# JCBrouwer/maua-style

Measured on AMD Instinct MI355X. Metric: optimizer iterations/sec at 1024x1024 VGG-19, higher is better.
Workload: dtype f32 (fp16x3 split-precision MFMA, fp32 accumulate)

## Files before the change

maua-style_amd/csrc/conv_x3p.hip:

```cpp
#include <stdlib.h>

#include <type_traits>

#include "conv_host.hpp"
#include "fp16x3.hpp"

namespace maua {

constexpr int XP_COT = 64;
constexpr int XP_ROWS = 16, XP_PR = 18, XP_PC = 34;
constexpr int XP_NPOS = XP_PR * XP_PC;
constexpr int XP_NPOS_PAD = 624;
constexpr int XP_PLANE = XP_NPOS_PAD * 16;
constexpr int XP_PATCH_BYTES = 8 * XP_PLANE;
constexpr int XP_TAP_BYTES = 2 * 4 * XP_COT * 16;
constexpr int XP_W_BYTES = 9 * XP_TAP_BYTES;
constexpr int XP_NI = 5;
constexpr int XP_THREADS = 512;
constexpr int XP_BIAS_MAX = 512;
constexpr int XP_LDS_BYTES = XP_PATCH_BYTES + XP_W_BYTES + 64 + XP_BIAS_MAX * 4 + XP_THREADS * 12;
constexpr unsigned XP_OOB = 0x80000000u;
#ifndef XP_W1_PIECES
#define XP_W1_PIECES 4
#endif
#ifndef XP_EARLY_LOADS
#define XP_EARLY_LOADS 0
#endif
#ifndef XP_MIDFOLD
#define XP_MIDFOLD 1
#endif
#ifndef XP_STAGGER
#define XP_STAGGER 0
#endif

__host__ __device__ constexpr int xp_first_pieces(bool pool) { return pool ? XP_W1_PIECES / 2 : XP_W1_PIECES; }
__host__ __device__ constexpr int xp_step_of(bool pool, int k) {
    const int p1 = xp_first_pieces(pool);
    return pool ? (k < p1 ? 16 - 2 * (p1 - 1 - k) : 20 + 2 * (k - p1)) : (k < p1 ? 17 - p1 + k : 20 + (k - p1));
}

struct X3pArgs {
    int items;
    int tiles;
    int ncot;
    int ksplit;
    int cps;
    int nmain;
    int n2;
    int groups;
    int tiles_y;
    int d_split, d_tx, d_ty, d_cot, d_n;
    int order;
    float w_inv_scale;
};

#ifdef XP_STAMP
#define XP_MARK(k)                                                                                                       \
    do {                                                                                                                 \
        if (lane == 0 && p.mask && chunk_no < 60) {                                                                      \
            const_cast<float*>(p.mask)[(((int64_t)blockIdx.x * 8 + wave) * 64 + chunk_no) * 8 + (k)] =                   \
                __builtin_bit_cast(float, (unsigned)__builtin_amdgcn_s_memtime());                                       \
        }                                                                                                                \
    } while (0)
#else
#define XP_MARK(k) do {} while (0)
#endif

#define XP_FENCE() __builtin_amdgcn_sched_barrier(0)

#define XP_PIPE_PLAIN(VA)                                             \
    do {                                                              \
        _Pragma("unroll") for (int m_ = 0; m_ < 12; ++m_) {           \
            __builtin_amdgcn_sched_group_barrier(0x008, 1, 0);        \
            __builtin_amdgcn_sched_group_barrier(0x100, 1, 0);        \
            __builtin_amdgcn_sched_group_barrier(0x020, 1, 0);        \
            __builtin_amdgcn_sched_group_barrier(0x200, 1, 0);        \
            __builtin_amdgcn_sched_group_barrier(0x002, VA, 0);       \
        }                                                             \
    } while (0)
#define XP_PIPE(VA)                                                   \
    do {                                                              \
        _Pragma("unroll") for (int m_ = 0; m_ < 12; ++m_) {           \
            __builtin_amdgcn_sched_group_barrier(0x008, 1, 0);        \
            __builtin_amdgcn_sched_group_barrier(0x100, 1, 0);        \
            __builtin_amdgcn_sched_group_barrier(0x020, 1, 0);        \
            __builtin_amdgcn_sched_group_barrier(0x040, 1, 0);        \
// ... 309 lines not shown
#pragma unroll
        for (int part = 0; part < 2; ++part) af[buf][part] = *reinterpret_cast<const f16x8*>(Wl + a_base + (tap * 2 + part) * 4096 + i * 256);
    };
    auto step_ = [&](auto stores, int tap, int i, int next_tap, auto fresh, float inv, auto va, auto&& extra) {
        constexpr bool FRESH = decltype(fresh)::value;
        constexpr int VA = decltype(va)::value;
        const int cur = i & 1;
        const bool refresh = i == 3 && next_tap >= 0;
        XP_FENCE();
        if (i < 3) load_ai(cur ^ 1, tap, i + 1);
        else if (next_tap >= 0 && tap != 4) load_ai(cur ^ 1, next_tap, 0);
        const f32x4 zero = {0.f, 0.f, 0.f, 0.f};
        if constexpr (FRESH) {
#pragma unroll
            for (int g = 0; g < 4; ++g) asm volatile("" : "+v"(acc[i][g]));
#pragma unroll
            for (int g = 0; g < 4; ++g)
#pragma unroll
                for (int r = 0; r < 4; ++r) master[i][g][r] = fmaf(acc[i][g][r], inv, master[i][g][r]);
#pragma unroll
            for (int g = 0; g < 4; ++g) asm volatile("" : "+v"(master[i][g]));
        }
#pragma unroll
        for (int g = 0; g < 4; ++g) acc[i][g] = __builtin_amdgcn_mfma_f32_16x16x32_f16(af[cur][1], bf[g][0], FRESH ? zero : acc[i][g], 0, 0, 0);
#pragma unroll
        for (int g = 0; g < 4; ++g) {
            acc[i][g] = __builtin_amdgcn_mfma_f32_16x16x32_f16(af[cur][0], bf[g][0], acc[i][g], 0, 0, 0);
            if (refresh) load_bg(g, 0, next_tap);
        }
        extra();
#pragma unroll
        for (int g = 0; g < 4; ++g) {
            acc[i][g] = __builtin_amdgcn_mfma_f32_16x16x32_f16(af[cur][0], bf[g][1], acc[i][g], 0, 0, 0);
            if (refresh) load_bg(g, 1, next_tap);
        }
        if constexpr (decltype(stores)::value) XP_PIPE(VA);
        else XP_PIPE_PLAIN(VA);
        XP_FENCE();
    };
    auto nothing = []() {};
    constexpr std::true_type FOLD{};
    constexpr std::false_type KEEP{};
    constexpr std::integral_constant<int, 0> V0{};
    constexpr std::integral_constant<int, 2> V2{};
    constexpr std::integral_constant<int, 4> V4{};

    Item cur = decode(item_begin);
    Item fin = cur;
    bool fin_valid = false;
    __amdgpu_buffer_rsrc_t rs_out, rs_aux;
    unsigned so_base = 0;
    unsigned vo[2];
    bool row_ok[4] = {true, true, true, true};
    const int PW = p.OW >> 1;
    const int pplane = (p.OH >> 1) * PW;
    auto epi_begin = [&]() {
        const int t_ = my_tid();
        const int lane = t_ & 63, px = t_ & 15, oct = (t_ >> 4) & 3, wave = wv;
        if constexpr (POOL) {
            const int64_t img = (int64_t)fin.n * p.Cout * pplane;
            rs_out = __builtin_amdgcn_make_buffer_rsrc(p.y + img, 0, (unsigned)p.Cout * (unsigned)pplane * 4u, 0x00020000);
            rs_aux = __builtin_amdgcn_make_buffer_rsrc(p.pool_codes + img, 0, (unsigned)p.Cout * (unsigned)pplane, 0x00020000);
            so_base = (unsigned)((fin.y0 >> 1) * PW + (fin.x0 >> 1));
#pragma unroll
            for (int h = 0; h < 2; ++h) {
                const int oy = fin.y0 + 2 * wave, oxx = fin.x0 + 16 * h + px;
                const bool store = fin_valid && (lane & 1) == 0 && oy + 1 < p.OH && oxx + 1 < p.OW;
                vo[h] = store ? (unsigned)(wave * PW + ((16 * h + px) >> 1)) : XP_OOB;
            }
        } else {
            const int64_t img = (int64_t)fin.n * p.Cout * out_plane;
            float* base = slab ? p.ws + ((int64_t)fin.n * ksplit + fin.split) * p.Cout * out_plane : p.y + img;
            rs_out = __builtin_amdgcn_make_buffer_rsrc(base, 0, (unsigned)p.Cout * (unsigned)out_plane * 4u, 0x00020000);
            rs_aux = rs_out;
            if constexpr (OM) rs_aux = __builtin_amdgcn_make_buffer_rsrc(const_cast<float*>(p.omask + img), 0, (unsigned)p.Cout * (unsigned)out_plane * 4u, 0x00020000);
            so_base = (unsigned)((fin.cot * XP_COT) * out_plane + fin.y0 * p.OW + fin.x0) * 4u;
#pragma unroll
            for (int h = 0; h < 2; ++h)
                vo[h] = fin_valid && fin.x0 + 16 * h + px < p.OW ? (unsigned)((4 * oct) * out_plane + (2 * wave) * p.OW + 16 * h + px) * 4u : XP_OOB;
#pragma unroll
            for (int g = 0; g < 4; ++g) row_ok[g] = fin.y0 + 2 * wv + (g >> 1) < p.OH;
        }
    };
    float mk[2][4];
    auto epi_load = [&](int k) {
        if constexpr (OM) {
            const int i = k >> 2, g = k & 3;
            const unsigned v = row_ok[g] ? vo[g & 1] : XP_OOB;
#pragma unroll
            for (int r = 0; r < 4; ++r)
                mk[k % 2][r] = __builtin_bit_cast(float, __builtin_amdgcn_raw_buffer_load_b32(
                    rs_aux, v, so_base + (unsigned)((16 * i + r) * out_plane + (g >> 1) * p.OW) * 4u, 0));
        }
    };
    auto reset_group = [&](int i, int cot) {
        const int oct = (my_tid() >> 4) & 3;
        const f32x4 b = *reinterpret_cast<const f32x4*>(Bl + cot * XP_COT + 16 * i + 4 * oct);
#pragma unroll
        for (int g = 0; g < 4; ++g) master[i][g] = b;
    };
    auto epi_piece = [&](int k, int next_cot) {
        const int oct = (my_tid() >> 4) & 3;
        if constexpr (POOL) {
            if (k >= 8) return;
            const int i = k >> 1, h = k & 1;
            unsigned pk = 0;
            const unsigned so = (unsigned)((fin.cot * XP_COT + 16 * i) * pplane) + so_base;
#pragma unroll
            for (int r = 0; r < 4; ++r) {
                float a = master[i][h][r], c = master[i][2 + h][r];
                a = a > 0.f ? a : 0.f;
                c = c > 0.f ? c : 0.f;
                const float b = __builtin_bit_cast(float, __builtin_amdgcn_update_dpp(0, __builtin_bit_cast(int, a), 0x101, 0xf, 0xf, false));
                const float d = __builtin_bit_cast(float, __builtin_amdgcn_update_dpp(0, __builtin_bit_cast(int, c), 0x101, 0xf, 0xf, false));
                float m = a;
                unsigned arg = 0;
                if (b > m) { m = b; arg = 1; }
                if (c > m) { m = c; arg = 2; }
                if (d > m) { m = d; arg = 3; }
                pk |= (arg | (m > 0.f ? 0u : 4u)) << (8 * r);
                const unsigned v = vo[h] == XP_OOB ? XP_OOB : ((unsigned)(4 * oct * pplane) + vo[h]) * 4u;
                __builtin_amdgcn_raw_buffer_store_b32(__builtin_bit_cast(unsigned, m), rs_out, v, (so + (unsigned)(r * pplane)) * 4u, 0);
            }
            const unsigned vc = vo[h] == XP_OOB ? XP_OOB : ((unsigned)((oct >> 1) * pplane) + vo[h]) * 8u + 4u * (oct & 1);
            __builtin_amdgcn_raw_buffer_store_b32(pk, rs_aux, vc, ((unsigned)(((fin.cot * XP_COT + 16 * i) >> 3) * pplane) + so_base) * 8u, 0);
            if (h == 1) reset_group(i, next_cot);
        } else {
            const int i = k >> 2, g = k & 3;
            const unsigned v = row_ok[g] ? vo[g & 1] : XP_OOB;
#pragma unroll
            for (int r = 0; r < 4; ++r) {
                float val = master[i][g][r];
                if (p.relu && !slab) val = val > 0.f ? val : 0.f;
                if constexpr (OM) val = mk[k % 2][r] > 0.f ? val : 0.f;
                __builtin_amdgcn_raw_buffer_store_b32(__builtin_bit_cast(unsigned, val), rs_out, v,
                                                      so_base + (unsigned)((16 * i + r) * out_plane + (g >> 1) * p.OW) * 4u, 0);
            }
            if (g == 3) reset_group(i, next_cot);
        }
    };

    auto gram_phase = [&](const Item& it, float inv_pending) {
#pragma unroll
        for (int i = 0; i < 4; ++i)
#pragma unroll
            for (int g = 0; g < 4; ++g)
#pragma unroll
                for (int r = 0; r < 4; ++r) {
                    master[i][g][r] = fmaf(acc[i][g][r], inv_pending, master[i][g][r]);
                    acc[i][g][r] = 0.f;
                }
        const float d_inv_scale = p.dinv[it.n];
        const unsigned char* dbank = reinterpret_cast<const unsigned char*>(p.dbank);
        unsigned vf[4];
#pragma unroll
        for (int g = 0; g < 4; ++g) {
            const int oy = it.y0 + 2 * wave + (g >> 1), oxx = it.x0 + (g & 1) * 16 + px;
            vf[g] = (oy < p.OH && oxx < p.OW) ? (unsigned)((oct * 8) * out_plane + oy * p.OW + oxx) * 4u : XP_OOB;
        }
        const unsigned frange = (unsigned)out_plane * 128u;
        float f[4][8];
        auto request = [&](int c2) {
            asm volatile("" : "+s"(c2));
            const __amdgpu_buffer_rsrc_t rs = __builtin_amdgcn_make_buffer_rsrc(
                const_cast<float*>(p.omask + ((int64_t)it.n * p.Cout + (int64_t)c2 * 32) * out_plane), 0, frange, 0x00020000);
#pragma unroll
            for (int c = 0; c < 8; ++c)
#pragma unroll
                for (int g = 0; g < 4; ++g) f[g][c] = __builtin_bit_cast(float, __builtin_amdgcn_raw_buffer_load_b32(rs, vf[g], c * out_plane * 4, 0));
        };
        request(0);
        for (int c2 = 0; c2 < q.n2; ++c2) {
            float m = 0.f;
#pragma unroll
            for (int g = 0; g < 4; ++g)
#pragma unroll
                for (int c = 0; c < 8; ++c) m = fmaxf(m, fabsf(f[g][c]));
            m = wave_max_nonneg(m);
            int e = (int)((__builtin_bit_cast(unsigned, m) >> 23) & 0xffu) - 127;
            e = m > 0.f ? max(e, -100) : 11;
            const float s = __builtin_bit_cast(float, (unsigned)(127 + 11 - e) << 23);
            const float inv = __builtin_bit_cast(float, (unsigned)(127 + e - 11) << 23) * d_inv_scale;
// ... 20 lines not shown
                for (int part = 0; part < 2; ++part) a[i][part] = *reinterpret_cast<const u32x4*>(gsrc + part * 2048 + i * 256);
            if (c2 + 1 < q.n2) request(c2 + 1);
#pragma unroll
            for (int i = 0; i < 4; ++i) {
                const f16x8 ah = __builtin_bit_cast(f16x8, a[i][0]), al = __builtin_bit_cast(f16x8, a[i][1]);
#pragma unroll
                for (int g = 0; g < 4; ++g) {
                    acc[i][g] = __builtin_amdgcn_mfma_f32_16x16x32_f16(al, b[g][0], acc[i][g], 0, 0, 0);
                    acc[i][g] = __builtin_amdgcn_mfma_f32_16x16x32_f16(ah, b[g][1], acc[i][g], 0, 0, 0);
                    acc[i][g] = __builtin_amdgcn_mfma_f32_16x16x32_f16(ah, b[g][0], acc[i][g], 0, 0, 0);
                }
            }
#pragma unroll
            for (int i = 0; i < 4; ++i)
#pragma unroll
                for (int g = 0; g < 4; ++g)
#pragma unroll
                    for (int r = 0; r < 4; ++r) {
                        master[i][g][r] = fmaf(acc[i][g][r], inv, master[i][g][r]);
                        acc[i][g][r] = 0.f;
                    }
        }
    };

    for (int c = tid; c < p.Cout; c += XP_THREADS) Bl[c] = (p.bias != nullptr && !slab) ? p.bias[c] : 0.f;
    set_tile(cur.x0, cur.y0);
    int ch = cur.cb;
    dma_filters(ch, cur.cot, 0, 9);
    if constexpr (!UNPOOL) voff[1] = Tl[2 * XP_THREADS + tid];
    load_patch_part(patch_rsrc(cur.n, ch), 0, 8);
    publish_max();
    asm volatile("s_waitcnt lgkmcnt(0)" ::: "memory");
    __builtin_amdgcn_s_barrier();
    float inv_prev = 0.f, inv_cur = 0.f, inv_next = 0.f;
    inv_cur = chunk_scale() * w_inv_scale;
    inv_next = inv_cur;
#pragma unroll
    for (int k = 0; k < NI; ++k) split_item(k);
    store_patch();
#pragma unroll
    for (int i = 0; i < 4; ++i) {
        reset_group(i, cur.cot);
#pragma unroll
        for (int g = 0; g < 4; ++g) acc[i][g] = f32x4{0.f, 0.f, 0.f, 0.f};
    }
    asm volatile("s_waitcnt vmcnt(0) lgkmcnt(0)" ::: "memory");
    __builtin_amdgcn_s_barrier();

#ifdef XP_STAMP
    int chunk_no = 0;
#endif
    auto chunk_body = [&](auto epi_tag, const Item& it, int chn, bool later, bool more, const Item& nx, int nch, const PatchSrc& rs) {
        constexpr bool EPI = decltype(epi_tag)::value;
        auto step = [&](int tap, int i, int next_tap, auto fresh, float inv, auto va, auto&& extra) {
            step_(std::integral_constant<bool, EPI>{}, tap, i, next_tap, fresh, inv, va, extra);
        };
        {
            const int t_ = my_tid();
            if constexpr (!UNPOOL) voff[1] = Tl[2 * XP_THREADS + t_];
            b_base = ((t_ >> 4) & 3) * XP_PLANE + ((2 * wv) * XP_PC + (t_ & 15)) * 16;
            a_base = ((t_ >> 4) & 3) * 1024 + (t_ & 15) * 16;
        }
        const int ncot_ = it.cot;
        if constexpr (EPI) epi_begin();
        constexpr int NP = POOL ? 8 : 16;
        constexpr int P1 = xp_first_pieces(POOL);
        auto step_of = [](int k) { return xp_step_of(POOL, k); };
        auto E = [&](int s) {
            if constexpr (EPI) {
#pragma unroll
                for (int k = 0; k < NP; ++k) {
                    if constexpr (OM) {
                        if (k < 1 ? s == step_of(0) - 1 : s == step_of(k - 1)) epi_load(k);
                    }
                }
#pragma unroll
                for (int k = 0; k < NP; ++k)
                    if (s == step_of(k) && fin_valid) epi_piece(k, ncot_);
            }
        };
        constexpr int SPP = POOL ? 5 : 4;
        constexpr int ST1 = !EPI ? 0 : SPP * P1;
        constexpr int late2 = POOL ? (NP - P1 > 3 ? NP - P1 - 3 : 0) : (NP - P1 > 5 ? NP - P1 - 5 : 0);
        constexpr int ST2 = !EPI ? 0 : SPP * late2;
        static_assert(ST1 <= 60 && ST2 <= 60 && xp_step_of(POOL, NP - 1) <= 31 && xp_step_of(POOL, 0) >= 5, "conv_x3p: epilogue schedule");
        constexpr std::integral_constant<int, EPI ? 4 : 2> VF{};
        constexpr std::integral_constant<int, EPI ? 2 : 0> VK{};
        XP_MARK(0);
#pragma unroll
        for (int g = 0; g < 4; ++g) {
            load_bg(g, 0, 0);
            load_bg(g, 1, 0);
        }
        load_ai(0, 0, 0);
        if constexpr (EPI || XP_EARLY_LOADS) {
            step(0, 0, 1, FOLD, inv_prev, VF, [&]() { load_patch_part(rs, 0, 1); });
            step(0, 1, 1, FOLD, inv_prev, VF, [&]() { load_patch_part(rs, 1, 2); if (later) dma_filters(chn, it.cot, 40, 1, 0); });
            step(0, 2, 1, FOLD, inv_prev, VF, [&]() { load_patch_part(rs, 2, 3); });
            step(0, 3, 1, FOLD, inv_prev, VF, [&]() { load_patch_part(rs, 3, 4); if (later) dma_filters(chn, it.cot, 40, 1, 1); });
            step(1, 0, 2, KEEP, 0.f, VK, [&]() { load_patch_part(rs, 4, 5); E(4); });
            step(1, 1, 2, KEEP, 0.f, VK, [&]() { load_patch_part(rs, 5, 6); if (later) dma_filters(chn, it.cot, 40, 1, 2); E(5); });
            step(1, 2, 2, KEEP, 0.f, VK, [&]() { load_patch_part(rs, 6, 7); E(6); });
            step(1, 3, 2, KEEP, 0.f, VK, [&]() { load_patch_part(rs, 7, 8); if (later) dma_filters(chn, it.cot, 40, 1, 3); E(7); });
#pragma unroll
            for (int tap = 2; tap < 4; ++tap)
#pragma unroll
                for (int i = 0; i < 4; ++i) step(tap, i, tap + 1, KEEP, 0.f, VK, [&]() { E(4 * tap + i); });
        } else {
            step(0, 0, 1, FOLD, inv_prev, VF, [&]() { load_patch_part(rs, 0, 1); });
            step(0, 1, 1, FOLD, inv_prev, VF, nothing);
            step(0, 2, 1, FOLD, inv_prev, VF, [&]() { load_patch_part(rs, 1, 2); });
            step(0, 3, 1, FOLD, inv_prev, VF, [&]() { if (later) dma_filters(chn, it.cot, 40, 1, 0); });
#pragma unroll
            for (int tap = 1; tap < 4; ++tap) {
                step(tap, 0, tap + 1, KEEP, 0.f, VK, [&]() { load_patch_part(rs, 2 * tap, 2 * tap + 1); });
                step(tap, 1, tap + 1, KEEP, 0.f, VK, nothing);
                step(tap, 2, tap + 1, KEEP, 0.f, VK, [&]() { load_patch_part(rs, 2 * tap + 1, 2 * tap + 2); });
                step(tap, 3, tap + 1, KEEP, 0.f, VK, [&]() { if (later) dma_filters(chn, it.cot, 40, 1, tap); });
            }
        }
        XP_MARK(1);
        step(4, 0, 5, KEEP, 0.f, VK, [&]() { E(16); });
        if (EPI && fin_valid) asm volatile("s_waitcnt vmcnt(%0)" ::"n"(ST1) : "memory");
        else asm volatile("s_waitcnt vmcnt(0)" ::: "memory");
        step(4, 1, 5, KEEP, 0.f, V4, [&]() { publish_max(); });
        step(4, 2, 5, KEEP, 0.f, V4, nothing);
        step(4, 3, 5, KEEP, 0.f, V0, nothing);
        XP_MARK(2);
        if (EPI && fin_valid) asm volatile("s_waitcnt vmcnt(%0) lgkmcnt(0)" ::"n"(ST1) : "memory");
        else asm volatile("s_waitcnt vmcnt(0) lgkmcnt(0)" ::: "memory");
        __builtin_amdgcn_s_barrier();
        XP_MARK(3);
        load_ai(0, 5, 0);
        inv_next = chunk_scale() * w_inv_scale;
// ... 35 lines not shown
        }
        XP_MARK(4);
        inv_prev = inv_cur;
        inv_cur = inv_next;
        asm volatile("s_waitcnt lgkmcnt(0)" ::: "memory");
        __builtin_amdgcn_s_barrier();
        XP_MARK(5);
        store_patch();
        if (EPI && fin_valid) asm volatile("s_waitcnt vmcnt(%0) lgkmcnt(0)" ::"n"(ST2) : "memory");
        else asm volatile("s_waitcnt vmcnt(0) lgkmcnt(0)" ::: "memory");
        __builtin_amdgcn_s_barrier();
        XP_MARK(6);
#ifdef XP_STAMP
        XP_MARK(7);
        ++chunk_no;
#endif
    };

    int item = item_begin;
    bool later = false;
    Item nx = cur;
    int nch = 0;
    bool more = true;
    PatchSrc rs;
    auto plan_next = [&](int chn) {
        const bool last_of_item = chn + 1 >= cur.ce;
        more = !(last_of_item && item + stride >= item_end);
        nx = cur;
        nch = chn + 1;
        if (last_of_item && more) {
            nx = advance(cur);
            nch = nx.cb;
            set_tile(nx.x0, nx.y0);
        }
        rs = patch_rsrc(more ? nx.n : cur.n, more ? nch : chn);
    };
    while (true) {
        plan_next(cur.cb);
        chunk_body(std::true_type{}, cur, cur.cb, later, more, nx, nch, rs);
        later = true;
        for (int chn = cur.cb + 1; chn < cur.ce; ++chn) {
            plan_next(chn);
            chunk_body(std::false_type{}, cur, chn, later, more, nx, nch, rs);
        }
        if constexpr (GRAM) {
            if (cur.split == ksplit - 1) {
                gram_phase(cur, inv_prev);
                inv_prev = 0.f;
            }
        }
        fin = cur;
        fin_valid = true;
        item += stride;
        if (!more) break;
        cur = nx;
    }
#pragma unroll
    for (int i = 0; i < 4; ++i)
#pragma unroll
        for (int g = 0; g < 4; ++g)
#pragma unroll
            for (int r = 0; r < 4; ++r) master[i][g][r] = fmaf(acc[i][g][r], inv_prev, master[i][g][r]);
    epi_begin();
    if constexpr (POOL) {
#pragma unroll
        for (int k = 0; k < 8; ++k) epi_piece(k, fin.cot);
    } else {
#pragma unroll
        for (int i = 0; i < 4; ++i) {
#pragma unroll
            for (int g = 0; g < 4; ++g) {
                epi_load(4 * i + g);
                epi_piece(4 * i + g, fin.cot);
            }
        }
    }
}


static int x3p_choose_split(const ConvArgs& a) {
    const int64_t items = conv_tiles(a, XP_ROWS) * ((a.Cout + XP_COT - 1) / XP_COT) * split_batch_hint();
    const int nchunks = a.Cin / 32;
    const int forced = (int)tuning("x3p_ks", 0);
    auto whole = [&](int ks) { const int cps = (nchunks + ks - 1) / ks; return (nchunks + cps - 1) / cps; };
    if (forced > 0) return whole(forced <= nchunks / 2 ? forced : (nchunks >= 4 ? nchunks / 2 : 1));
    if (items >= 512 || nchunks < 4) return 1;
    const double out_mb = (double)split_batch_hint() * a.Cout * a.OH * a.OW * 4.0 / 1e6;
    int best = 1;
    double best_cost = 1e30;
    for (int ks = 1; ks <= 16 && ks <= nchunks / 2; ++ks) {
        const int64_t its = items * ks;
        const double per_wg = (double)((its + 255) / 256);
        double cost = (per_wg * (double)((nchunks + ks - 1) / ks) + 0.7) * 9.0;
        if (ks > 1) cost += (ks + 1) * out_mb / 5.0 + 5.0;
        if (cost < best_cost * 0.97) {
            best_cost = cost;
            best = ks;
        }
    }
    return whole(best);
}

bool conv_x3p_supports(const ConvArgs& a) {
    return a.Cin % 32 == 0 && a.Cout % XP_COT == 0 && a.Cout <= XP_BIAS_MAX && (int64_t)a.H * a.W <= (1ll << 24) && a.pad >= 0 && a.pad <= 2 &&
           (int64_t)a.Cout * a.OH * a.OW * 4 < (1ll << 31) && (int64_t)a.OH * a.OW <= (1ll << 24);
}

static int g_xp_max_groups = 0;
static int x3p_max_groups() {
    const int v = g_xp_max_groups > 0 ? g_xp_max_groups : (int)tuning("x3p_groups", 256);
    return v >= 8 ? v / 8 * 8 : 256;
}

#ifdef XP_STAMP
static float* g_xp_stamp = nullptr;
extern "C" void maua_xp_set_stamp_buffer(float* buf) { g_xp_stamp = buf; }
#endif

template <bool OM, bool POOL, bool UNPOOL, bool GRAM>
static int xp_launch_one(const ConvArgs& p, const X3pArgs& q, hipStream_t stream) {
    const void* fn = reinterpret_cast<const void*>(&conv_x3p_kernel<OM, POOL, UNPOOL, GRAM>);
    static unsigned long long served = 0;
    const hipError_t rc = opt_in_dynamic_lds(fn, XP_LDS_BYTES, &served);
    if (rc != hipSuccess) {
        set_error("conv_x3p: hipFuncSetAttribute: %s", hipGetErrorString(rc));
        return (int)rc;
    }
    hipLaunchKernelGGL((conv_x3p_kernel<OM, POOL, UNPOOL, GRAM>), dim3((unsigned)q.groups), dim3(XP_THREADS), XP_LDS_BYTES, stream, p, q);
    return check_launch("conv_x3p_kernel");
// ... 146 lines not shown
```

maua-style_amd/csrc/conv_x3q.hip:

```cpp
#include <stdlib.h>

#include <type_traits>

#include "conv_host.hpp"
#include "fp16x3.hpp"

namespace maua {

constexpr int XQ_COT = 64;
constexpr int XQ_ROWS = 16, XQ_PR = 18, XQ_PC = 34;
constexpr int XQ_NPOS = XQ_PR * XQ_PC;
constexpr int XQ_NPOS_PAD = 624;
constexpr int XQ_PLANE = XQ_NPOS_PAD * 16;
constexpr int XQ_PATCH_BYTES = 8 * XQ_PLANE;
constexpr int XQ_TAP_BYTES = 2 * 4 * XQ_COT * 16;
constexpr int XQ_W_BYTES = 9 * XQ_TAP_BYTES;
constexpr int XQ_ITEMS = 4 * XQ_NPOS;
constexpr int XQ_NI = 5;
constexpr int XQ_THREADS = 512;
constexpr int XQ_LDS_BYTES = XQ_PATCH_BYTES + XQ_W_BYTES + 64;

__global__ void pack_x3q_kernel(const float* __restrict__ w, unsigned short* __restrict__ bank, int cout, int cin, int backward,
                                float w_scale) {
    const int CO = backward ? cin : cout;
    const int CI = backward ? cout : cin;
    const int nchunk = (CI + 31) / 32, ntile = (CO + XQ_COT - 1) / XQ_COT;
    const int64_t total = (int64_t)nchunk * ntile * 9 * 4 * XQ_COT * 8;
    for (int64_t e = (int64_t)blockIdx.x * blockDim.x + threadIdx.x; e < total; e += (int64_t)gridDim.x * blockDim.x) {
        int64_t r = e;
        const int ch = (int)(r % 8);
        r /= 8;
        const int co = (int)(r % XQ_COT);
        r /= XQ_COT;
        const int oct = (int)(r % 4);
        r /= 4;
        const int tap = (int)(r % 9);
        r /= 9;
        const int tile = (int)(r % ntile);
        const int chunk = (int)(r / ntile);
        const int o = tile * XQ_COT + co, i = chunk * 32 + oct * 8 + ch;
        float v = 0.f;
        if (o < CO && i < CI) {
            if (!backward) v = w[((int64_t)o * cin + i) * 9 + tap];
            else v = w[((int64_t)i * cin + o) * 9 + (8 - tap)];
        }
        v *= w_scale;
        const _Float16 h = (_Float16)v;
        const _Float16 l = (_Float16)(v - (float)h);
        const int64_t base = ((int64_t)chunk * ntile + tile) * (XQ_W_BYTES / 2);
        bank[base + ((((int64_t)tap * 2 + 0) * 4 + oct) * XQ_COT + co) * 8 + ch] = __builtin_bit_cast(unsigned short, h);
        bank[base + ((((int64_t)tap * 2 + 1) * 4 + oct) * XQ_COT + co) * 8 + ch] = __builtin_bit_cast(unsigned short, l);
    }
}

#ifdef XQ_STAMP
#define XQ_MARK(k)                                                                                          \
    do {                                                                                                    \
        if (lane == 0 && p.mask) {                                                                          \
            const unsigned long long t_ = __builtin_amdgcn_s_memtime();                                     \
            const_cast<float*>(p.mask)[((((int64_t)blockIdx.y * gridDim.x + blockIdx.x) * 8 + wave) * 64 + (ch - ch_begin)) * 8 + (k)] = \
                __builtin_bit_cast(float, (unsigned)t_);                                                    \
        }                                                                                                   \
    } while (0)
#else
#define XQ_MARK(k) do {} while (0)
#endif

#define XQ_FENCE() __builtin_amdgcn_sched_barrier(0)

__device__ __forceinline__ const ConvArgs* xq_kernel_arguments() {
#if defined(__HIP_DEVICE_COMPILE__)
    return (const ConvArgs*)__builtin_amdgcn_kernarg_segment_ptr();
#else
// ... 118 lines not shown
        PatchSrc r;
        r.x = __builtin_amdgcn_make_buffer_rsrc(const_cast<float*>(xin + (int64_t)ch * 32 * st_plane), 0, range, 0x00020000);
        r.codes = r.x;
        if constexpr (UNPOOL)
            r.codes = __builtin_amdgcn_make_buffer_rsrc(const_cast<unsigned char*>(xcodes + (int64_t)ch * 32 * st_plane), 0, range >> 2, 0x00020000);
        return r;
    };
    auto load_patch_part = [&](const PatchSrc& rs, int c_lo, int c_hi) {
#ifdef XQ_NO_SPLIT
#if defined(__HIP_DEVICE_COMPILE__)
        for (int c = c_lo; c < c_hi; ++c)
            if (c < 5)
                for (int part = 0; part < 2; ++part)
                    __builtin_amdgcn_raw_ptr_buffer_load_lds(rs.x, (__attribute__((address_space(3))) void*)(Pl + ((wv * 5 + c) * 2 + part) * 992), 16,
                                                             voff[c < NI ? c : 0], part * 64, 0, 0);
#endif
        return;
#endif
        if constexpr (UNPOOL) {
            if (c_lo == 0) {
#pragma unroll
                for (int k = 0; k < NI; ++k) cd[k] = __builtin_amdgcn_raw_buffer_load_b64(rs.codes, vcode[k], 0, 0);
            }
        }
#pragma unroll
        for (int c = c_lo; c < c_hi; ++c)
#pragma unroll
            for (int k = 0; k < NI; ++k)
                rp[k][c] = __builtin_bit_cast(float, __builtin_amdgcn_raw_buffer_load_b32(rs.x, voff[k], c * st_plane * 4, 0));
    };
    auto publish_max = [&]() {
#ifdef XQ_NO_SPLIT
        if (lane == 0) Ml[wave] = 1.f;
        return;
#endif
        if constexpr (UNPOOL) {
            const unsigned m2 = code_mask * 0x00010001u;
#pragma unroll
            for (int k = 0; k < NI; ++k)
#pragma unroll
                for (int i = 0; i < 4; ++i) {
                    sel2[k][i] = __builtin_amdgcn_perm(0u, cd[k][i >> 1], (i & 1) ? 0x0c030c02u : 0x0c010c00u) & m2;
                    const unsigned s0 = sel2[k][i] & 0xffffu, s1 = sel2[k][i] >> 16;
                    rp[k][2 * i] = ((inmask[k] >> s0) & 1u) ? rp[k][2 * i] : 0.f;
                    rp[k][2 * i + 1] = ((inmask[k] >> s1) & 1u) ? rp[k][2 * i + 1] : 0.f;
                }
        }
        float m = 0.f;
#pragma unroll
        for (int k = 0; k < NI; ++k)
#pragma unroll
            for (int c = 0; c < 8; ++c) m = fmaxf(m, fabsf(rp[k][c]));
        m = wave_max_nonneg(m);
        if (lane == 0) Ml[wave] = m;
    };
    float sx = 1.f;
    auto chunk_scale = [&]() {
        const float m = fmaxf(fmaxf(fmaxf(Ml[0], Ml[1]), fmaxf(Ml[2], Ml[3])), fmaxf(fmaxf(Ml[4], Ml[5]), fmaxf(Ml[6], Ml[7])));
        int e = (int)((__builtin_bit_cast(unsigned, m) >> 23) & 0xffu) - 127;
        e = m > 0.f ? max(e, -100) : 11;
        sx = __builtin_bit_cast(float, (unsigned)(127 + 11 - e) << 23);
        return __builtin_bit_cast(float, (unsigned)(127 + e - 11) << 23);
    };
    auto split_item = [&](int k) {
#ifdef XQ_NO_SPLIT
        return;
#endif
        if (k >= NI) return;
#pragma unroll
        for (int c = 0; c < 8; ++c) asm volatile("" : "+v"(rp[k][c]));
        unsigned hu[4], lu[4];
#pragma unroll
        for (int q = 0; q < 4; ++q) {
            const float v0 = rp[k][2 * q], v1 = rp[k][2 * q + 1];
            const f16x2 h2 = {(_Float16)(v0 * sx), (_Float16)(v1 * sx)};
            const f16x2 l2 = {(_Float16)fmaf(v0, sx, -(float)h2[0]), (_Float16)fmaf(v1, sx, -(float)h2[1])};
            hu[q] = __builtin_bit_cast(unsigned, h2);
            lu[q] = __builtin_bit_cast(unsigned, l2);
        }
#pragma unroll
        for (int q = 0; q < 4; ++q) {
            rp[k][q] = __builtin_bit_cast(float, hu[q]);
            rp[k][4 + q] = __builtin_bit_cast(float, lu[q]);
        }
#pragma unroll
        for (int c = 0; c < 8; ++c) asm volatile("" : "+v"(rp[k][c]));
    };
    auto store_patch = [&]() {
#ifdef XQ_NO_SPLIT
        return;
#endif
        if constexpr (UNPOOL) {
#pragma unroll
            for (int k = 0; k < NI; ++k)
#pragma unroll
                for (int q = 0; q < 4; ++q)
                    if ((inmask[k] >> q) & 1u) {
                        const unsigned dst = lds_w[k] + (unsigned)(((q >> 1) * XQ_PC + (q & 1)) * 16);
                        u32x4 h, l;
#pragma unroll
                        for (int i = 0; i < 4; ++i) {
                            const unsigned t = sel2[k][i] ^ ((unsigned)q * 0x00010001u);
                            const unsigned keep = ((t & 0xffffu) ? 0u : 0xffffu) | ((t >> 16) ? 0u : 0xffff0000u);
                            h[i] = __builtin_bit_cast(unsigned, rp[k][i]) & keep;
                            l[i] = __builtin_bit_cast(unsigned, rp[k][4 + i]) & keep;
                        }
                        *reinterpret_cast<u32x4*>(Pl + dst) = h;
// ... 256 lines not shown
                }
            }
        }
#pragma unroll
        for (int i = 0; i < 4; ++i)
#pragma unroll
            for (int r = 0; r < 4; ++r) {
                const int co = co0 + i * 16 + 4 * oct + r;
                const float b0 = bias != nullptr ? bias[min(co, kp->Cout - 1)] : 0.f;
#pragma unroll
                for (int g = 0; g < 4; ++g) master[i][g][r] = acc[i][g][r] + b0;
            }
        final_sums = true;
    }
    if constexpr (POOL) if (final_sums) {
        const int PW = p.OW >> 1;
        const int64_t pplane = (int64_t)(p.OH >> 1) * PW;
        float* __restrict__ py = p.y + (int64_t)n * p.Cout * pplane;
        unsigned char* __restrict__ pc = p.pool_codes + (int64_t)n * p.Cout * pplane;
        const int oy = y0 + 2 * wave;
#pragma unroll
        for (int h = 0; h < 2; ++h) {
            const int oxx = x0 + 16 * h + px;
            const bool store = (lane & 1) == 0 && oy + 1 < p.OH && oxx + 1 < p.OW;
            const int64_t ppix = (int64_t)(oy >> 1) * PW + (oxx >> 1);
#pragma unroll
            for (int i = 0; i < 4; ++i) {
                const int cq = co0 + 16 * i + 4 * oct;
                unsigned pk = 0;
#pragma unroll
                for (int r = 0; r < 4; ++r) {
                    float a = master[i][h][r], c = master[i][2 + h][r];
                    a = a > 0.f ? a : 0.f;
                    c = c > 0.f ? c : 0.f;
                    const float b = __builtin_bit_cast(float, __builtin_amdgcn_update_dpp(0, __builtin_bit_cast(int, a), 0x101, 0xf, 0xf, false));
                    const float d = __builtin_bit_cast(float, __builtin_amdgcn_update_dpp(0, __builtin_bit_cast(int, c), 0x101, 0xf, 0xf, false));
                    float m = a;
                    unsigned arg = 0;
                    if (b > m) { m = b; arg = 1; }
                    if (c > m) { m = c; arg = 2; }
                    if (d > m) { m = d; arg = 3; }
                    pk |= (arg | (m > 0.f ? 0u : 4u)) << (8 * r);
                    if (store && cq < p.Cout) py[(int64_t)(cq + r) * pplane + ppix] = m;
                }
                if (store && cq < p.Cout) *reinterpret_cast<unsigned*>(pc + ((int64_t)(cq >> 3) * pplane + ppix) * 8 + (cq & 7)) = pk;
            }
        }
        XQ_EXIT_STAMP();
        return;
    }
    float* __restrict__ yout = p.y + (int64_t)n * p.Cout * out_plane;
    const float* __restrict__ om = p.omask ? p.omask + (int64_t)n * p.Cout * out_plane : nullptr;
    const bool full = co0 + XQ_COT <= p.Cout;
#pragma unroll
    for (int g = 0; g < 4; ++g) {
        const int oy = y0 + 2 * wave + (g >> 1), ox = x0 + (g & 1) * 16 + px;
        const bool pvalid = oy < p.OH && ox < p.OW;
        const int64_t opix = (int64_t)oy * p.OW + ox;
        if (!final_sums) {
            float* wsp = p.ws + (int64_t)blockIdx.z * p.Cout * out_plane;
#pragma unroll
            for (int i = 0; i < 4; ++i)
#pragma unroll
                for (int r = 0; r < 4; ++r) {
                    const int co = co0 + i * 16 + 4 * oct + r;
                    if (pvalid && co < p.Cout) wsp[(int64_t)co * out_plane + opix] = master[i][g][r];
                }
            continue;
        }
        XQ_FENCE();
        if (!pvalid) continue;
        const int cl = co0 + 4 * oct;
        int64_t lane_off = (int64_t)cl * out_plane + opix;
        if constexpr (ACC || OM) asm volatile("" : "+v"(lane_off));
        float* __restrict__ yl = yout + lane_off;
        const float* __restrict__ oml = OM ? om + lane_off : nullptr;
        constexpr int GB = ACC ? 1 : 4;
#pragma unroll
        for (int i0 = 0; i0 < 4; i0 += GB) {
            if constexpr (ACC) XQ_FENCE();
            float prev[GB * 4], msk[GB * 4];
#pragma unroll
            for (int i = i0; i < i0 + GB; ++i)
#pragma unroll
                for (int r = 0; r < 4; ++r) {
                    const int cr = i * 16 + r, e = (i - i0) * 4 + r;
                    const bool cv = full || cl + cr < p.Cout;
                    prev[e] = 0.f;
                    msk[e] = 1.f;
                    if constexpr (ACC) if (cv) prev[e] = yl[(int64_t)cr * out_plane];
                    if constexpr (OM) if (cv) msk[e] = oml[(int64_t)cr * out_plane];
                }
#pragma unroll
            for (int i = i0; i < i0 + GB; ++i)
#pragma unroll
                for (int r = 0; r < 4; ++r) {
                    const int cr = i * 16 + r, e = (i - i0) * 4 + r;
                    float v = master[i][g][r] + prev[e];
                    if (p.relu) v = v > 0.f ? v : 0.f;
                    v = msk[e] > 0.f ? v : 0.f;
                    if (full || cl + cr < p.Cout) yl[(int64_t)cr * out_plane] = v;
                }
        }
    }
    XQ_EXIT_STAMP();
}
// ... 157 lines not shown
```

maua-style_amd/csrc/fp16x3.hpp:

```cpp
#pragma once
#include "common.hpp"

namespace maua {

typedef float f32x16 __attribute__((ext_vector_type(16)));
typedef float f32x4 __attribute__((ext_vector_type(4)));
typedef float f32x2 __attribute__((ext_vector_type(2)));
typedef _Float16 f16x8 __attribute__((ext_vector_type(8)));
typedef _Float16 f16x4 __attribute__((ext_vector_type(4)));
typedef _Float16 f16x2 __attribute__((ext_vector_type(2)));
typedef __attribute__((ext_vector_type(4))) unsigned int u32x4;
typedef __attribute__((ext_vector_type(2))) unsigned int u32x2;

__device__ __forceinline__ unsigned cvt_pk_f16(float a, float b) {
    const f32x2 v = {a, b};
    return __builtin_bit_cast(unsigned, __builtin_convertvector(v, f16x2));
}
__device__ __forceinline__ float f16_lo(unsigned u) { return (float)__builtin_bit_cast(f16x2, u)[0]; }
__device__ __forceinline__ float f16_hi(unsigned u) { return (float)__builtin_bit_cast(f16x2, u)[1]; }

}
```

Before: 200.0.

## Widen conv epilogue stores to 128-bit via quad DPP transpose

Adds a wide epilogue path to the x3p and x3q conv kernels. When OW is a multiple of 4 and the output pointers are 16-byte aligned, each group of 4 lanes transposes its accumulator fragment with DPP swaps, so a lane holds 4 consecutive pixels of one channel. It then issues one 128-bit store (and 128-bit mask load) in place of four scalar 32-bit accesses. In x3p, when wide mode is active, the epilogue runs on its own after each item instead of interleaved with the MMA steps, and the epilogue step spacing constant changes. This trades some compute/epilogue overlap and extra DPP ops for fewer, wider memory transactions.

```diff
diff --git a/maua-style_amd/csrc/conv_x3p.hip b/maua-style_amd/csrc/conv_x3p.hip
--- a/maua-style_amd/csrc/conv_x3p.hip
+++ b/maua-style_amd/csrc/conv_x3p.hip
@@ -32,6 +32,9 @@
 #ifndef XP_STAGGER
 #define XP_STAGGER 0
 #endif
+#ifndef XP_WIDE_EPI
+#define XP_WIDE_EPI 1
+#endif
 
 __host__ __device__ constexpr int xp_first_pieces(bool pool) { return pool ? XP_W1_PIECES / 2 : XP_W1_PIECES; }
 __host__ __device__ constexpr int xp_step_of(bool pool, int k) {
@@ -447,6 +450,13 @@
     unsigned so_base = 0;
     unsigned vo[2];
     bool row_ok[4] = {true, true, true, true};
+    constexpr bool WIDE_EPI = XP_WIDE_EPI != 0 && !POOL && !UNPOOL && !GRAM;
+    bool wide = false;
+    if constexpr (WIDE_EPI) {
+        size_t al = reinterpret_cast<size_t>(slab ? p.ws : p.y);
+        if constexpr (OM) al |= reinterpret_cast<size_t>(p.omask);
+        wide = (p.OW & 3) == 0 && (al & 15) == 0;
+    }
     const int PW = p.OW >> 1;
     const int pplane = (p.OH >> 1) * PW;
     auto epi_begin = [&]() {
@@ -471,17 +481,32 @@
             if constexpr (OM) rs_aux = __builtin_amdgcn_make_buffer_rsrc(const_cast<float*>(p.omask + img), 0, (unsigned)p.Cout * (unsigned)out_plane * 4u, 0x00020000);
             so_base = (unsigned)((fin.cot * XP_COT) * out_plane + fin.y0 * p.OW + fin.x0) * 4u;
 #pragma unroll
-            for (int h = 0; h < 2; ++h)
+            for (int h = 0; h < 2; ++h) {
                 vo[h] = fin_valid && fin.x0 + 16 * h + px < p.OW ? (unsigned)((4 * oct) * out_plane + (2 * wave) * p.OW + 16 * h + px) * 4u : XP_OOB;
+                if constexpr (WIDE_EPI) {
+                    const unsigned vw = fin_valid && fin.x0 + 16 * h + (px & 12) < p.OW
+                                            ? (unsigned)((4 * oct + (px & 3)) * out_plane + (2 * wave) * p.OW + 16 * h + (px & 12)) * 4u : XP_OOB;
+                    vo[h] = wide ? vw : vo[h];
+                }
+            }
 #pragma unroll
             for (int g = 0; g < 4; ++g) row_ok[g] = fin.y0 + 2 * wv + (g >> 1) < p.OH;
         }
     };
     float mk[2][4];
-    auto epi_load = [&](int k) {
+    auto epi_load = [&](int k, auto wtag) {
         if constexpr (OM) {
             const int i = k >> 2, g = k & 3;
             const unsigned v = row_ok[g] ? vo[g & 1] : XP_OOB;
+            if constexpr (WIDE_EPI) {
+                if constexpr (decltype(wtag)::value) {
+                    const f32x4 m4 = __builtin_bit_cast(
+                        f32x4, __builtin_amdgcn_raw_buffer_load_b128(rs_aux, v, so_base + (unsigned)((16 * i) * out_plane + (g >> 1) * p.OW) * 4u, 0));
+#pragma unroll
+                    for (int r = 0; r < 4; ++r) mk[k % 2][r] = m4[r];
+                    return;
+                }
+            }
 #pragma unroll
             for (int r = 0; r < 4; ++r)
                 mk[k % 2][r] = __builtin_bit_cast(float, __builtin_amdgcn_raw_buffer_load_b32(
@@ -494,7 +519,7 @@
 #pragma unroll
         for (int g = 0; g < 4; ++g) master[i][g] = b;
     };
-    auto epi_piece = [&](int k, int next_cot) {
+    auto epi_piece = [&](int k, int next_cot, auto wtag) {
         const int oct = (my_tid() >> 4) & 3;
         if constexpr (POOL) {
             if (k >= 8) return;
@@ -523,6 +548,23 @@
         } else {
             const int i = k >> 2, g = k & 3;
             const unsigned v = row_ok[g] ? vo[g & 1] : XP_OOB;
+            if constexpr (WIDE_EPI) {
+                if constexpr (decltype(wtag)::value) {
+                    const int t_ = my_tid();
+                    f32x4 w4 = __builtin_bit_cast(f32x4, quad_transpose(__builtin_bit_cast(u32x4, master[i][g]), t_));
+#pragma unroll
+                    for (int r = 0; r < 4; ++r) {
+                        float val = w4[r];
+                        if (p.relu && !slab) val = val > 0.f ? val : 0.f;
+                        if constexpr (OM) val = mk[k % 2][r] > 0.f ? val : 0.f;
+                        w4[r] = val;
+                    }
+                    const unsigned so = so_base + (unsigned)((16 * i) * out_plane + (g >> 1) * p.OW) * 4u;
+                    __builtin_amdgcn_raw_buffer_store_b128(__builtin_bit_cast(u32x4, w4), rs_out, v + so, 0, 0);
+                    if (g == 3) reset_group(i, next_cot);
+                    return;
+                }
+            }
 #pragma unroll
             for (int r = 0; r < 4; ++r) {
                 float val = master[i][g][r];
@@ -649,6 +691,7 @@
 #endif
     auto chunk_body = [&](auto epi_tag, const Item& it, int chn, bool later, bool more, const Item& nx, int nch, const PatchSrc& rs) {
         constexpr bool EPI = decltype(epi_tag)::value;
+        constexpr std::integral_constant<bool, WIDE_EPI> wtag{};
         auto step = [&](int tap, int i, int next_tap, auto fresh, float inv, auto va, auto&& extra) {
             step_(std::integral_constant<bool, EPI>{}, tap, i, next_tap, fresh, inv, va, extra);
         };
@@ -668,15 +711,15 @@
 #pragma unroll
                 for (int k = 0; k < NP; ++k) {
                     if constexpr (OM) {
-                        if (k < 1 ? s == step_of(0) - 1 : s == step_of(k - 1)) epi_load(k);
+                        if (k < 1 ? s == step_of(0) - 1 : s == step_of(k - 1)) epi_load(k, wtag);
                     }
                 }
 #pragma unroll
                 for (int k = 0; k < NP; ++k)
-                    if (s == step_of(k) && fin_valid) epi_piece(k, ncot_);
+                    if (s == step_of(k) && fin_valid) epi_piece(k, ncot_, wtag);
             }
         };
-        constexpr int SPP = POOL ? 5 : 4;
+        constexpr int SPP = POOL ? 5 : (WIDE_EPI && decltype(wtag)::value ? 1 : 4);
         constexpr int ST1 = !EPI ? 0 : SPP * P1;
         constexpr int late2 = POOL ? (NP - P1 > 3 ? NP - P1 - 3 : 0) : (NP - P1 > 5 ? NP - P1 - 5 : 0);
         constexpr int ST2 = !EPI ? 0 : SPP * late2;
@@ -818,9 +861,48 @@
         fin = cur;
         fin_valid = true;
         item += stride;
+#if XP_WIDE_EPI
+        if ((WIDE_EPI && !wide) || !more) {
+#pragma unroll
+            for (int i = 0; i < 4; ++i)
+#pragma unroll
+                for (int g = 0; g < 4; ++g)
+#pragma unroll
+                    for (int r = 0; r < 4; ++r) {
+                        master[i][g][r] = fmaf(acc[i][g][r], inv_prev, master[i][g][r]);
+                        acc[i][g][r] = -0.f;
+                    }
+            inv_prev = 1.f;
+            epi_begin();
+            const int next_cot = more ? nx.cot : fin.cot;
+            auto alone = [&](auto wtag) {
+                if constexpr (POOL) {
+#pragma unroll
+                    for (int k = 0; k < 8; ++k) epi_piece(k, next_cot, wtag);
+                } else {
+#pragma unroll
+                    for (int i = 0; i < 4; ++i) {
+#pragma unroll
+                        for (int g = 0; g < 4; ++g) {
+                            epi_load(4 * i + g, wtag);
+                            epi_piece(4 * i + g, next_cot, wtag);
+                        }
+                    }
+                }
+            };
+            if constexpr (WIDE_EPI) {
+                if (wide) alone(std::true_type{});
+                else alone(std::false_type{});
+            } else {
+                alone(std::false_type{});
+            }
+            fin_valid = false;
+        }
+#endif
         if (!more) break;
         cur = nx;
     }
+#if !XP_WIDE_EPI
 #pragma unroll
     for (int i = 0; i < 4; ++i)
 #pragma unroll
@@ -830,17 +912,18 @@
     epi_begin();
     if constexpr (POOL) {
 #pragma unroll
-        for (int k = 0; k < 8; ++k) epi_piece(k, fin.cot);
+        for (int k = 0; k < 8; ++k) epi_piece(k, fin.cot, std::false_type{});
     } else {
 #pragma unroll
         for (int i = 0; i < 4; ++i) {
 #pragma unroll
             for (int g = 0; g < 4; ++g) {
-                epi_load(4 * i + g);
-                epi_piece(4 * i + g, fin.cot);
+                epi_load(4 * i + g, std::false_type{});
+                epi_piece(4 * i + g, fin.cot, std::false_type{});
             }
         }
     }
+#endif
 }
 
 
diff --git a/maua-style_amd/csrc/conv_x3q.hip b/maua-style_amd/csrc/conv_x3q.hip
--- a/maua-style_amd/csrc/conv_x3q.hip
+++ b/maua-style_amd/csrc/conv_x3q.hip
@@ -19,6 +19,9 @@
 constexpr int XQ_NI = 5;
 constexpr int XQ_THREADS = 512;
 constexpr int XQ_LDS_BYTES = XQ_PATCH_BYTES + XQ_W_BYTES + 64;
+#ifndef XQ_WIDE_EPI
+#define XQ_WIDE_EPI 1
+#endif
 
 __global__ void pack_x3q_kernel(const float* __restrict__ w, unsigned short* __restrict__ bank, int cout, int cin, int backward,
                                 float w_scale) {
@@ -243,7 +246,11 @@
 #pragma unroll
             for (int c = 0; c < 8; ++c) m = fmaxf(m, fabsf(rp[k][c]));
         m = wave_max_nonneg(m);
+#if XQ_WIDE_EPI
+        if (lane == 0) Ml[wv] = m;
+#else
         if (lane == 0) Ml[wave] = m;
+#endif
     };
     float sx = 1.f;
     auto chunk_scale = [&]() {
@@ -606,6 +613,69 @@
     float* __restrict__ yout = p.y + (int64_t)n * p.Cout * out_plane;
     const float* __restrict__ om = p.omask ? p.omask + (int64_t)n * p.Cout * out_plane : nullptr;
     const bool full = co0 + XQ_COT <= p.Cout;
+#if XQ_WIDE_EPI
+    bool wide;
+    {
+        size_t al = reinterpret_cast<size_t>(final_sums ? kp->y : kp->ws);
+        if constexpr (OM) al |= reinterpret_cast<size_t>(kp->omask);
+        wide = (kp->OW & 3) == 0 && (al & 15) == 0;
+    }
+    if (wide) {
+        int t_ = wv * 64 + (int)__builtin_amdgcn_mbcnt_hi(~0u, __builtin_amdgcn_mbcnt_lo(~0u, 0u));
+        asm volatile("" : "+v"(t_));
+        const int pq = t_ & 12, tq = t_ & 3;
+        const int oct = (t_ >> 4) & 3, wave = __builtin_amdgcn_readfirstlane(t_ >> 6);
+        const int cl = co0 + 4 * oct + tq;
+#pragma unroll
+        for (int g = 0; g < 4; ++g) {
+            const int oy = y0 + 2 * wave + (g >> 1), ox = x0 + (g & 1) * 16 + pq;
+            const bool pvalid = oy < p.OH && ox < p.OW;
+            int64_t lane_off = (int64_t)cl * out_plane + (int64_t)oy * p.OW + ox;
+            XQ_FENCE();
+            asm volatile("" : "+v"(lane_off));
+            if (!final_sums) {
+                float* wsl = p.ws + (int64_t)blockIdx.z * p.Cout * out_plane + lane_off;
+#pragma unroll
+                for (int i = 0; i < 4; ++i) {
+                    const u32x4 w4 = quad_transpose(__builtin_bit_cast(u32x4, master[i][g]), t_);
+                    if (pvalid && cl + 16 * i < p.Cout) *reinterpret_cast<u32x4*>(wsl + (int64_t)(16 * i) * out_plane) = w4;
+                }
+                continue;
+            }
+            float* __restrict__ yl = yout + lane_off;
+            const float* __restrict__ oml = OM ? om + lane_off : nullptr;
+            constexpr int GB = ACC ? 1 : 4;
+#pragma unroll
+            for (int i0 = 0; i0 < 4; i0 += GB) {
+                if constexpr (ACC) XQ_FENCE();
+                f32x4 prev[GB], msk[GB];
+#pragma unroll
+                for (int i = i0; i < i0 + GB; ++i) {
+                    const bool cv = pvalid && (full || cl + 16 * i < p.Cout);
+                    prev[i - i0] = f32x4{0.f, 0.f, 0.f, 0.f};
+                    msk[i - i0] = f32x4{1.f, 1.f, 1.f, 1.f};
+                    if constexpr (ACC) if (cv) prev[i - i0] = *reinterpret_cast<const f32x4*>(yl + (int64_t)(16 * i) * out_plane);
+                    if constexpr (OM) if (cv) msk[i - i0] = *reinterpret_cast<const f32x4*>(oml + (int64_t)(16 * i) * out_plane);
+                }
+#pragma unroll
+                for (int i = i0; i < i0 + GB; ++i) {
+                    const f32x4 t4 = __builtin_bit_cast(f32x4, quad_transpose(__builtin_bit_cast(u32x4, master[i][g]), t_));
+                    f32x4 o4;
+#pragma unroll
+                    for (int r = 0; r < 4; ++r) {
+                        float v = t4[r] + prev[i - i0][r];
+                        if (p.relu) v = v > 0.f ? v : 0.f;
+                        v = msk[i - i0][r] > 0.f ? v : 0.f;
+                        o4[r] = v;
+                    }
+                    if (pvalid && (full || cl + 16 * i < p.Cout)) *reinterpret_cast<f32x4*>(yl + (int64_t)(16 * i) * out_plane) = o4;
+                }
+            }
+        }
+        XQ_EXIT_STAMP();
+        return;
+    }
+#endif
 #pragma unroll
     for (int g = 0; g < 4; ++g) {
         const int oy = y0 + 2 * wave + (g >> 1), ox = x0 + (g & 1) * 16 + px;
diff --git a/maua-style_amd/csrc/fp16x3.hpp b/maua-style_amd/csrc/fp16x3.hpp
--- a/maua-style_amd/csrc/fp16x3.hpp
+++ b/maua-style_amd/csrc/fp16x3.hpp
@@ -16,6 +16,22 @@
     const f32x2 v = {a, b};
     return __builtin_bit_cast(unsigned, __builtin_convertvector(v, f16x2));
 }
+__device__ __forceinline__ u32x4 quad_transpose(u32x4 v, int lane) {
+#if defined(__HIP_DEVICE_COMPILE__)
+    const bool odd = (lane & 1) != 0, hi = (lane & 2) != 0;
+    auto swap1 = [](unsigned x) { return (unsigned)__builtin_amdgcn_update_dpp(0, (int)x, 0xB1, 0xf, 0xf, false); };
+    auto swap2 = [](unsigned x) { return (unsigned)__builtin_amdgcn_update_dpp(0, (int)x, 0x4E, 0xf, 0xf, false); };
+    const unsigned x0 = swap1(v[0]), x1 = swap1(v[1]), x2 = swap1(v[2]), x3 = swap1(v[3]);
+    const unsigned a0 = odd ? x1 : v[0], a1 = odd ? v[1] : x0, a2 = odd ? x3 : v[2], a3 = odd ? v[3] : x2;
+    const unsigned y0 = swap2(a0), y1 = swap2(a1), y2 = swap2(a2), y3 = swap2(a3);
+    const u32x4 b = {hi ? y2 : a0, hi ? y3 : a1, hi ? a2 : y0, hi ? a3 : y1};
+    return b;
+#else
+    (void)lane;
+    return v;
+#endif
+}
+
 __device__ __forceinline__ float f16_lo(unsigned u) { return (float)__builtin_bit_cast(f16x2, u)[0]; }
 __device__ __forceinline__ float f16_hi(unsigned u) { return (float)__builtin_bit_cast(f16x2, u)[1]; }
 
```

Result: no change. 198.7 (-0.6%).
